# TengdaHan/TemporalAlignNet

Hardware: AMD Instinct MI355X
Metric: video-seq/sec (len=64, E6D6) at 1/2/4/8 MI355X; HTM-Align ROC-AUC parity (higher is better)
Workload: dtype bf16; 1 GPU; E6D6 len=64 bf16 stage-1 (init: multi-positive NCE only) train step (fwd+loss+bwd+AdamW), synthetic HTM-370K-shaped features, N~U[4,16] sentences/video; global_batch=128, per_gpu_batch=128, seq_len=64, parallelism=dp1

## Files before the change

temporalalignnet_amd/csrc/tan_attnblk.hip:

```cpp
#include "tan_panel.h"
#include "tan_attn_img.h"

namespace tal {

typedef float f32x4_t __attribute__((ext_vector_type(4)));

struct AbFwdArgs {
    const bf16_t* xn1; const bf16_t* x_in; const unsigned char* keypad;
    const char* pw_qkv;
    const char* pw_out;
    const float* b_qkv; const float* b_out;
    bf16_t* qkv; bf16_t* attn_o; float* lse;
    bf16_t* x_mid;
    int L, H;
    long long* dbg;
    float* part; long part_plane;
};

constexpr int AB_D = 4;
struct AbWFrags { bf16x8 f[3]; };

__device__ __forceinline__ void ab_load_wa(AbWFrags& W, const char* pw, int hp, int ks, int wave, int lane) {
    const char* p = pw + ((long)((hp * 16 + ks) * PN_WAVES + wave) * 3) * 1024 + lane * 16;
#pragma unroll
    for (int i = 0; i < 3; ++i) W.f[i] = *reinterpret_cast<const bf16x8*>(p + i * 1024);
}
__device__ __forceinline__ void ab_load_wb(AbWFrags& W, const char* pw, int kt, int wave, int lane) {
    const char* p = pw + (long)kt * 16384 + wave * 2048 + lane * 16;
#pragma unroll
    for (int i = 0; i < 2; ++i) W.f[i] = *reinterpret_cast<const bf16x8*>(p + i * 1024);
}

template <int NKB>
__device__ __forceinline__ float ab_attn_unit(char* Qi, const char* Ki, const char* Vi, const float* bias, int q0, int lane) {
    const int c = lane & 31, hh = lane >> 5;
    bf16x8 qf[4];
#pragma unroll
    for (int ks = 0; ks < 4; ++ks) qf[ks] = img_frag_kc(Qi, q0 + c, 2 * ks + hh);
    f32x16 s[NKB];
    float m = -INFINITY;
#pragma unroll
    for (int kb = 0; kb < NKB; ++kb) {
        acc_zero(s[kb]);
#pragma unroll
        for (int ks = 0; ks < 4; ++ks)
            s[kb] = __builtin_amdgcn_mfma_f32_32x32x16_bf16(img_frag_kc(Ki, 32 * kb + c, 2 * ks + hh), qf[ks], s[kb], 0, 0, 0);
#pragma unroll
        for (int g4 = 0; g4 < 4; ++g4) {
            const float4 bv = *reinterpret_cast<const float4*>(bias + 32 * kb + 8 * g4 + 4 * hh);
            const float bb[4] = {bv.x, bv.y, bv.z, bv.w};
#pragma unroll
            for (int e = 0; e < 4; ++e) {
                const float v = s[kb][4 * g4 + e] * 0.125f + bb[e];
                s[kb][4 * g4 + e] = v;
                m = fmaxf(m, v);
            }
        }
    }
    m = fmaxf(m, __shfl_xor(m, 32, 64));
    const bool dead = (m == -INFINITY);
    float sum = 0.f;
#pragma unroll
    for (int kb = 0; kb < NKB; ++kb)
#pragma unroll
        for (int r = 0; r < 16; ++r) {
            const float e = dead ? 0.f : __expf(s[kb][r] - m);
            s[kb][r] = e;
            sum += e;
        }
    sum += __shfl_xor(sum, 32, 64);
    const float inv = dead ? 0.f : 1.0f / sum;
    f32x16 o[2];
    acc_zero(o[0]); acc_zero(o[1]);
#pragma unroll
    for (int kb = 0; kb < NKB; ++kb) {
#pragma unroll
        for (int r = 0; r < 16; ++r) s[kb][r] *= inv;
#pragma unroll
        for (int j = 0; j < 2; ++j) {
            const bf16x8 pf = acc_frag(s[kb], j);
#pragma unroll
            for (int db = 0; db < 2; ++db)
                o[db] = __builtin_amdgcn_mfma_f32_32x32x16_bf16(img_frag_tr(Vi, 32 * kb + 16 * j, 32 * db, lane), pf, o[db], 0, 0, 0);
        }
    }
#pragma unroll
    for (int db = 0; db < 2; ++db)
#pragma unroll
        for (int g4 = 0; g4 < 4; ++g4) {
            const int row = q0 + c, chunk = 4 * db + g4;
            st4((bf16_t*)(Qi + row * 128 + ((chunk ^ img_swz(row)) << 4) + hh * 8),
                make_float4(o[db][4 * g4], o[db][4 * g4 + 1], o[db][4 * g4 + 2], o[db][4 * g4 + 3]));
        }
    return dead ? -INFINITY : m + logf(sum);
}

__device__ __forceinline__ void ab_rows_out(const char* img, int r0, int lane, bf16_t* out, long ld, int L) {
#pragma unroll
    for (int it = 0; it < 4; ++it) {
        const int row = r0 + it * 8 + (lane >> 3), chunk = lane & 7;
        const uint4 v = *reinterpret_cast<const uint4*>(img + row * 128 + ((chunk ^ img_swz(row)) << 4));
        if (row < L) *reinterpret_cast<uint4*>(out + (long)row * ld + chunk * 8) = v;
    }
}

template <int NRB16, bool SPLIT = false>
__global__ __launch_bounds__(64 * PN_WAVES, PN_WAVES / 4) void attnblk_fwd_kernel(AbFwdArgs a) {
    static_assert(PN_WAVES == 8, "eight waves");
    constexpr int NKB = (NRB16 + 1) / 2, LP = 32 * NKB, XROWS = 16 * NRB16, D = AB_D;
    constexpr int XP_OFF = 0, IMG_OFF = XROWS * 1024, IMG_B = LP * 128, BIAS_OFF = IMG_OFF + 6 * IMG_B, BQ_OFF = BIAS_OFF + LP * 4, LDS_B = BQ_OFF + 1536 * 4;
    static_assert(LDS_B <= 163840, "LDS budget");
    __shared__ __attribute__((aligned(1024))) char lds[LDS_B];

    const int tid = threadIdx.x, lane = tid & 63, hi = lane >> 5;
    const int wave = __builtin_amdgcn_readfirstlane(tid >> 6);
    const int L = a.L, C = 512;
    const long row0 = (long)blockIdx.x * L;
    const char* const pwa = a.pw_qkv;
    const char* const pwb = a.pw_out;
    const int hp0 = SPLIT ? (int)blockIdx.y : 0, hp1 = SPLIT ? hp0 + 1 : 4;

    AbWFrags WQ[D];
    pn_static_for<0, D>([&](auto jc) {
        constexpr int J = decltype(jc)::value;
        ab_load_wa(WQ[J], pwa, hp0, J, wave, lane);
    });

    {
        constexpr int RPW = XROWS / PN_WAVES;
        uint4 v[RPW];
#pragma unroll
        for (int r = 0; r < RPW; ++r) {
            const int m = wave * RPW + r;
            v[r] = *reinterpret_cast<const uint4*>(a.xn1 + (row0 + min(m, L - 1)) * C + lane * 8);
        }
#pragma unroll
        for (int r = 0; r < RPW; ++r) *reinterpret_cast<uint4*>(pn_panel_slot<1024>(lds + XP_OFF, wave * RPW + r, lane)) = v[r];
        float* bias = reinterpret_cast<float*>(lds + BIAS_OFF);
        const unsigned char* kp = a.keypad ? a.keypad + (long)blockIdx.x * L : nullptr;
        for (int j = tid; j < LP; j += 64 * PN_WAVES) bias[j] = (j >= L || (kp && kp[j])) ? -INFINITY : 0.f;
        for (int j = tid; j < 1536 / 4; j += 64 * PN_WAVES)
            reinterpret_cast<float4*>(lds + BQ_OFF)[j] = reinterpret_cast<const float4*>(a.b_qkv)[j];
        if constexpr (LP > XROWS) {
            constexpr int PER = (LP - XROWS) * 8;
            for (int i = tid; i < 6 * PER; i += 64 * PN_WAVES)
                *reinterpret_cast<uint4*>(lds + IMG_OFF + (i / PER) * IMG_B + XROWS * 128 + (i % PER) * 16) = make_uint4(0, 0, 0, 0);
        }
    }
    __syncthreads();

    f32x16 acc_o[2][NKB];
#pragma unroll
    for (int i = 0; i < 2; ++i)
#pragma unroll
        for (int j = 0; j < NKB; ++j) acc_zero(acc_o[i][j]);

    typedef __attribute__((address_space(3))) const bf16x8* lds_frag_t;
    const float* bias = reinterpret_cast<const float*>(lds + BIAS_OFF);
    const bool saving = a.qkv != nullptr;

    constexpr int PPI = LP / 8, NPW = 2 * PPI / PN_WAVES;
    constexpr int NIDLE = PN_WAVES - 2 * NKB, NKV = 4 * PPI / NIDLE;
    static_assert(2 * PPI % PN_WAVES == 0 && 4 * PPI % NIDLE == 0, "piece split");
    uint4 cpv;
    auto copy_read = [&](int i, int ln) __attribute__((always_inline)) {
        const int g = wave + PN_WAVES * i, j = g / PPI, row = (g % PPI) * 8 + (ln >> 3), chunk = ln & 7;
        cpv = *reinterpret_cast<const uint4*>(lds + IMG_OFF + (j * 3) * IMG_B + row * 128 + ((chunk ^ img_swz(row)) << 4));
    };
    auto copy_store = [&](int i, int ln, int hp_prev) __attribute__((always_inline)) {
        const int g = wave + PN_WAVES * i, j = g / PPI, row = (g % PPI) * 8 + (ln >> 3), chunk = ln & 7;
        if (row < L) *reinterpret_cast<uint4*>(a.attn_o + (row0 + row) * C + (2 * hp_prev + j) * 64 + chunk * 8) = cpv;
    };

    f32x4_t acc_a[3][NRB16];
    auto gemm_a = [&](int hp, auto copy_flag) __attribute__((always_inline)) {
        constexpr bool COPY = decltype(copy_flag)::value;
        int ln = lane;
        asm volatile("" : "+v"(ln));
        const int xrow = ln & 15, xq = ln >> 4;
        const unsigned xbase = (unsigned)(uintptr_t)(lds + XP_OFF + xrow * 1024);
#pragma unroll
        for (int fb = 0; fb < 3; ++fb) {
            const int p = 3 * wave + fb, which = (p >> 2) % 3, j = p / 12, fblk = p & 3;
            const float4 bv = *reinterpret_cast<const float4*>(lds + BQ_OFF + (which * C + (2 * hp + j) * 64 + fblk * 16 + 4 * xq) * 4);
#pragma unroll
            for (int rb = 0; rb < NRB16; ++rb) { acc_a[fb][rb][0] = bv.x; acc_a[fb][rb][1] = bv.y; acc_a[fb][rb][2] = bv.z; acc_a[fb][rb][3] = bv.w; }
        }
        bf16x8 X[NRB16];
#pragma unroll
        for (int rb = 0; rb < NRB16; ++rb) X[rb] = *(lds_frag_t)(uintptr_t)(xbase + rb * 16384 + ((xq ^ xrow) << 4));
        __builtin_amdgcn_sched_barrier(0);
        pn_static_for<0, 16>([&](auto jc) {
            constexpr int KS = decltype(jc)::value;
            AbWFrags& W = WQ[KS % D];
            if constexpr (COPY) {
                if (saving) {
                    if constexpr (KS >= 1 && KS <= NPW) copy_store(KS - 1, ln, hp - 1);
                    if constexpr (KS < NPW) copy_read(KS, ln);
                }
            }
#pragma unroll
            for (int rb = 0; rb < NRB16; ++rb) {
#pragma unroll
                for (int fb = 0; fb < 3; ++fb)
                    acc_a[fb][rb] = __builtin_amdgcn_mfma_f32_16x16x32_bf16(W.f[fb], X[rb], acc_a[fb][rb], 0, 0, 0);
                if constexpr (KS < 15) X[rb] = *(lds_frag_t)(uintptr_t)(xbase + rb * 16384 + ((((KS + 1) * 4 + xq) ^ xrow) << 4));
            }
            if constexpr (KS + D < 16) ab_load_wa(W, pwa, hp, KS + D, wave, ln);
            else ab_load_wb(W, pwb, hp * 8 + (KS + D - 16), wave, ln);
            __builtin_amdgcn_sched_barrier(0);
        });
    };

    gemm_a(hp0, std::false_type{});
#pragma unroll 1
    for (int hp = hp0; hp < hp1; ++hp) {
        __syncthreads();
        {
            int ln = lane;
            asm volatile("" : "+v"(ln));
            const int erow = ln & 15, eq = ln >> 4;
#pragma unroll
            for (int fb = 0; fb < 3; ++fb) {
                const int p = 3 * wave + fb, which = (p >> 2) % 3, j = p / 12, fblk = p & 3;
                char* img = lds + IMG_OFF + (j * 3 + which) * IMG_B;
#pragma unroll
                for (int rb = 0; rb < NRB16; ++rb) {
                    const int row = rb * 16 + erow, chunk = fblk * 2 + (eq >> 1);
                    uint2 u;
                    u.x = f2bf2(acc_a[fb][rb][0], acc_a[fb][rb][1]);
                    u.y = f2bf2(acc_a[fb][rb][2], acc_a[fb][rb][3]);
                    *reinterpret_cast<uint2*>(img + row * 128 + ((chunk ^ img_swz(row)) << 4) + (eq & 1) * 8) = u;
                }
            }
        }
        __syncthreads();

        if (wave >= 2 * NKB) {
            if (saving) {
                int ln = lane;
                asm volatile("" : "+v"(ln));
#pragma unroll 4
                for (int i = 0; i < NKV; ++i) {
                    const int g = (wave - 2 * NKB) + NIDLE * i, im = g / PPI, j = im >> 1, which = 1 + (im & 1);
                    const int row = (g % PPI) * 8 + (ln >> 3), chunk = ln & 7;
                    const uint4 v = *reinterpret_cast<const uint4*>(lds + IMG_OFF + (j * 3 + which) * IMG_B + row * 128 + ((chunk ^ img_swz(row)) << 4));
                    if (row < L) *reinterpret_cast<uint4*>(a.qkv + (row0 + row) * (3 * C) + which * C + (2 * hp + j) * 64 + chunk * 8) = v;
                }
            }
        } else {
            int ln = lane;
            asm volatile("" : "+v"(ln));
            const int j = wave / NKB, q0 = (wave % NKB) * 32, h = 2 * hp + j;
            char* Qi = lds + IMG_OFF + (j * 3) * IMG_B;
            if (saving) ab_rows_out(Qi, q0, ln, a.qkv + row0 * (3 * C) + h * 64, 3 * C, L);
            const float l = ab_attn_unit<NKB>(Qi, Qi + IMG_B, Qi + 2 * IMG_B, bias, q0, ln);
            if (saving && ln < 32 && q0 + ln < L) a.lse[((long)blockIdx.x * a.H + h) * L + q0 + ln] = l;
        }
        __syncthreads();

        {
            int ln = lane;
            asm volatile("" : "+v"(ln));
            pn_static_for<0, 8>([&](auto jc) {
                constexpr int KB = decltype(jc)::value;
                const char* Oi = lds + IMG_OFF + ((KB >> 2) * 3) * IMG_B;
                AbWFrags& W = WQ[KB % D];
                bf16x8 of[NKB];
#pragma unroll
                for (int rb = 0; rb < NKB; ++rb) of[rb] = img_frag_kc(Oi, rb * 32 + (ln & 31), 2 * (KB & 3) + (ln >> 5));
#pragma unroll
                for (int nb = 0; nb < 2; ++nb)
#pragma unroll
                    for (int rb = 0; rb < NKB; ++rb)
                        acc_o[nb][rb] = __builtin_amdgcn_mfma_f32_32x32x16_bf16(W.f[nb], of[rb], acc_o[nb][rb], 0, 0, 0);
                if constexpr (KB + D < 8) ab_load_wb(W, pwb, hp * 8 + KB + D, wave, ln);
                else if (hp + 1 < hp1) ab_load_wa(W, pwa, hp + 1, KB + D - 8, wave, ln);
                __builtin_amdgcn_sched_barrier(0);
            });
        }
        if (hp + 1 < hp1) gemm_a(hp + 1, std::true_type{});
    }
    if constexpr (SPLIT) {
        if (saving) {
#pragma unroll 1
            for (int i = 0; i < NPW; ++i) { copy_read(i, lane); copy_store(i, lane, hp0); }
        }
#pragma unroll
        for (int nb = 0; nb < 2; ++nb)
#pragma unroll
            for (int mb = 0; mb < NKB; ++mb) {
                const int m = mb * 32 + (lane & 31);
                if (m < L) {
                    float* dst = a.part + hp0 * a.part_plane + (row0 + m) * C + wave * 64 + nb * 32 + 16 * hi;
#pragma unroll
                    for (int q = 0; q < 4; ++q)
                        *reinterpret_cast<float4*>(dst + 4 * q) = make_float4(acc_o[nb][mb][4 * q], acc_o[nb][mb][4 * q + 1], acc_o[nb][mb][4 * q + 2],
                                                                              acc_o[nb][mb][4 * q + 3]);
                }
            }
        return;
    }
    uint4 resq[2][NKB][2];
#pragma unroll
    for (int nb = 0; nb < 2; ++nb)
#pragma unroll
        for (int mb = 0; mb < NKB; ++mb)
#pragma unroll
            for (int p = 0; p < 2; ++p)
                resq[nb][mb][p] = *reinterpret_cast<const uint4*>(a.x_in + (row0 + min(mb * 32 + (lane & 31), L - 1)) * C + wave * 64 + nb * 32 + (2 * hi + p) * 8);
    if (saving) {
#pragma unroll 1
        for (int i = 0; i < NPW; ++i) { copy_read(i, lane); copy_store(i, lane, 3); }
    }

    __syncthreads();
    char* xo_panel = lds + XP_OFF;
#pragma unroll
    for (int nb = 0; nb < 2; ++nb) {
        const int nbase = wave * 64 + nb * 32;
        pn_cfptr_t bp = (pn_cfptr_t)(uintptr_t)(a.b_out) + nbase;
#pragma unroll
        for (int mb = 0; mb < NKB; ++mb) {
            const int m = mb * 32 + (lane & 31);
#pragma unroll
            for (int p = 0; p < 2; ++p) {
                float bias8[8], res[8], v[8];
                pn_uniform8(bp + 8 * p, bp + 16 + 8 * p, hi, bias8);
                pn_unpack8(resq[nb][mb][p], res);
#pragma unroll
                for (int e = 0; e < 8; ++e) v[e] = acc_o[nb][mb][8 * p + e] + bias8[e] + res[e];
                if (m < XROWS) *reinterpret_cast<uint4*>(pn_panel_slot<1024>(xo_panel, m, (nbase >> 3) + 2 * hi + p)) = pn_pack8(v);
            }
        }
    }
    __syncthreads();
    for (int m = wave; m < L; m += PN_WAVES)
        *reinterpret_cast<uint4*>(a.x_mid + (row0 + m) * C + lane * 8) = *reinterpret_cast<const uint4*>(pn_panel_slot<1024>(xo_panel, m, lane));
}

__global__ __launch_bounds__(256) void attnblk_split_finish_kernel(const float* __restrict__ part, long plane, const bf16_t* __restrict__ x_in,
                                                                   const float* __restrict__ b_out, bf16_t* __restrict__ x_mid, long rows) {
    const int lane = threadIdx.x & 63, wave = threadIdx.x >> 6;
    const long row = (long)blockIdx.x * 4 + wave;
    if (row >= rows) return;
    f8 acc = ld8f(part + row * 512 + lane * 8);
#pragma unroll
    for (int c = 1; c < 4; ++c) {
        const f8 t = ld8f(part + c * plane + row * 512 + lane * 8);
#pragma unroll
        for (int j = 0; j < 8; ++j) acc.v[j] += t.v[j];
    }
    const f8 res = ld8(x_in + row * 512 + lane * 8), bias = ld8f(b_out + lane * 8);
    f8 v;
#pragma unroll
    for (int j = 0; j < 8; ++j) v.v[j] = acc.v[j] + bias.v[j] + res.v[j];
    st8(x_mid + row * 512 + lane * 8, v);
}

}

using namespace tal;

static long long* g_ab_dbg = nullptr;
extern "C" int tan_attnblk_lab_set_dbg(void* p) { g_ab_dbg = (long long*)p; return 0; }

extern "C" int tan_attnblk_supported(int L, int C, int H, int dtype) {
    return dtype == TAN_BF16 && C == 512 && H == 8 && L > 48 && L <= 80;
}

extern "C" int tan_attnblk_fwd(const tan_attnblk_desc* d, void* stream) {
    TAN_REQUIRE(d && d->xn1 && d->x_in && d->pw_qkv && d->pw_out && d->b_qkv && d->b_out && d->x_mid && d->B > 0);
    TAN_REQUIRE(tan_attnblk_supported(d->L, d->C, d->H, TAN_BF16));
    TAN_REQUIRE((d->qkv != nullptr) == (d->attn_o != nullptr) && (d->qkv != nullptr) == (d->lse != nullptr));
    AbFwdArgs a;
    a.xn1 = (const bf16_t*)d->xn1; a.x_in = (const bf16_t*)d->x_in; a.keypad = d->key_padding_mask;
    a.pw_qkv = (const char*)d->pw_qkv; a.pw_out = (const char*)d->pw_out; a.b_qkv = d->b_qkv; a.b_out = d->b_out;
    a.qkv = (bf16_t*)d->qkv; a.attn_o = (bf16_t*)d->attn_o; a.lse = d->lse; a.x_mid = (bf16_t*)d->x_mid;
    a.L = d->L; a.H = d->H; a.dbg = g_ab_dbg;
    a.part = nullptr; a.part_plane = 0;
    const dim3 grid((unsigned)d->B);
    const double rows = (double)d->B * d->L;
    const int rec = prof_begin((hipStream_t)stream, TAN_PROF_ATTNBLK, 2.0 * rows * 512.0 * 2048.0 + 4.0 * rows * d->L * 512.0);
    if (d->L <= 64) hipLaunchKernelGGL((attnblk_fwd_kernel<4>), grid, dim3(64 * PN_WAVES), 0, (hipStream_t)stream, a);
    else hipLaunchKernelGGL((attnblk_fwd_kernel<5>), grid, dim3(64 * PN_WAVES), 0, (hipStream_t)stream, a);
    prof_end((hipStream_t)stream, rec);
    TAN_LAUNCH_CHECK();
    return 0;
}

extern "C" int tan_attnblk_fwd_split(const tan_attnblk_desc* d, float* part, void* stream) {
    TAN_REQUIRE(d && part && d->xn1 && d->x_in && d->pw_qkv && d->pw_out && d->b_qkv && d->b_out && d->x_mid && d->B > 0);
    TAN_REQUIRE(tan_attnblk_supported(d->L, d->C, d->H, TAN_BF16));
    TAN_REQUIRE((d->qkv != nullptr) == (d->attn_o != nullptr) && (d->qkv != nullptr) == (d->lse != nullptr));
    AbFwdArgs a;
    a.xn1 = (const bf16_t*)d->xn1; a.x_in = (const bf16_t*)d->x_in; a.keypad = d->key_padding_mask;
    a.pw_qkv = (const char*)d->pw_qkv; a.pw_out = (const char*)d->pw_out; a.b_qkv = d->b_qkv; a.b_out = d->b_out;
    a.qkv = (bf16_t*)d->qkv; a.attn_o = (bf16_t*)d->attn_o; a.lse = d->lse; a.x_mid = (bf16_t*)d->x_mid;
    a.L = d->L; a.H = d->H; a.dbg = nullptr;
    const long rows = (long)d->B * d->L;
    a.part = part; a.part_plane = rows * 512;
    const hipStream_t st = (hipStream_t)stream;
    const dim3 grid((unsigned)d->B, 4);
    const int rec = prof_begin(st, TAN_PROF_ATTNBLK, 2.0 * rows * 512.0 * 2048.0 + 4.0 * rows * d->L * 512.0);
    if (d->L <= 64) hipLaunchKernelGGL((attnblk_fwd_kernel<4, true>), grid, dim3(64 * PN_WAVES), 0, st, a);
    else hipLaunchKernelGGL((attnblk_fwd_kernel<5, true>), grid, dim3(64 * PN_WAVES), 0, st, a);
    prof_end(st, rec);
    TAN_LAUNCH_CHECK();
    hipLaunchKernelGGL(attnblk_split_finish_kernel, dim3(cdiv(rows, 4)), dim3(256), 0, st, part, rows * 512, (const bf16_t*)d->x_in, d->b_out,
                       (bf16_t*)d->x_mid, rows);
    TAN_LAUNCH_CHECK();
    return 0;
}
```

Measured before the change: 31550 video-seq/s.

## Add warp-specialized pipelined attention block kernel overlapping QKV GEMM with attention

Adds a new fused attention-block forward kernel that splits the eight waves into producer and consumer groups. Four waves compute the next head's QKV projection into double-buffered LDS images while the other four run attention for the current head, then all waves accumulate the output projection. Weight fragments for the next stage are prefetched inside the MFMA loops. The new kernel is enabled by default through an environment flag, and it adds LDS pressure and per-head barriers.

```diff
diff --git a/temporalalignnet_amd/csrc/tan_attnblk.hip b/temporalalignnet_amd/csrc/tan_attnblk.hip
--- a/temporalalignnet_amd/csrc/tan_attnblk.hip
+++ b/temporalalignnet_amd/csrc/tan_attnblk.hip
@@ -339,6 +339,226 @@
         *reinterpret_cast<uint4*>(a.x_mid + (row0 + m) * C + lane * 8) = *reinterpret_cast<const uint4*>(pn_panel_slot<1024>(xo_panel, m, lane));
 }
 
+template <int NRB16, bool CLK = false>
+__global__ __launch_bounds__(64 * PN_WAVES, PN_WAVES / 4) void attnblk_fwd_pipe_kernel(AbFwdArgs a) {
+    static_assert(PN_WAVES == 8, "eight waves");
+    constexpr int NKB = (NRB16 + 1) / 2, LP = 32 * NKB, XROWS = 16 * NRB16, D = AB_D, NH = 8;
+    constexpr int XP_OFF = 0, IMG_OFF = XROWS * 1024, IMG_B = LP * 128, BIAS_OFF = IMG_OFF + 6 * IMG_B, BQ_OFF = BIAS_OFF + LP * 4, LDS_B = BQ_OFF + 1536 * 4;
+    static_assert(LDS_B <= 163840, "LDS budget");
+    __shared__ __attribute__((aligned(1024))) char lds[LDS_B];
+
+    const int tid = threadIdx.x, lane = tid & 63, hi = lane >> 5;
+    const int wave = __builtin_amdgcn_readfirstlane(tid >> 6);
+    const bool gw = wave < 4;
+    const int rw = wave & 3;
+    const int L = a.L, C = 512;
+    const long row0 = (long)blockIdx.x * L;
+    const char* const pwa = a.pw_qkv;
+    const char* const pwb = a.pw_out;
+    auto clk = [&](int i) __attribute__((always_inline)) {
+        if constexpr (CLK) {
+            if (blockIdx.x == 0 && lane == 0) a.dbg[wave * 32 + i] = (long long)__builtin_amdgcn_s_memtime();
+        }
+    };
+    clk(0);
+    auto load_wa = [&](AbWFrags& W, int h, int ks, int ln) __attribute__((always_inline)) { ab_load_wa(W, pwa, h >> 1, ks, 4 * (h & 1) + rw, ln); };
+
+    auto load_sel = [&](AbWFrags& W, bool in, int h, int ks, int kt, int ln) __attribute__((always_inline)) {
+        const char* p = in ? pwa + ((long)(((h >> 1) * 16 + ks) * PN_WAVES + 4 * (h & 1) + rw) * 3) * 1024 : pwb + (long)kt * 16384 + wave * 2048;
+        p += ln * 16;
+        const int o2 = in ? 2048 : 1024;
+        W.f[0] = *reinterpret_cast<const bf16x8*>(p);
+        W.f[1] = *reinterpret_cast<const bf16x8*>(p + 1024);
+        W.f[2] = *reinterpret_cast<const bf16x8*>(p + o2);
+    };
+
+    AbWFrags WQ[D];
+    pn_static_for<0, D>([&](auto jc) { load_sel(WQ[decltype(jc)::value], gw, 0, decltype(jc)::value, decltype(jc)::value, lane); });
+
+    {
+        constexpr int RPW = XROWS / PN_WAVES;
+        uint4 v[RPW];
+#pragma unroll
+        for (int r = 0; r < RPW; ++r) {
+            const int m = wave * RPW + r;
+            v[r] = *reinterpret_cast<const uint4*>(a.xn1 + (row0 + min(m, L - 1)) * C + lane * 8);
+        }
+#pragma unroll
+        for (int r = 0; r < RPW; ++r) *reinterpret_cast<uint4*>(pn_panel_slot<1024>(lds + XP_OFF, wave * RPW + r, lane)) = v[r];
+        float* bias = reinterpret_cast<float*>(lds + BIAS_OFF);
+        const unsigned char* kp = a.keypad ? a.keypad + (long)blockIdx.x * L : nullptr;
+        for (int j = tid; j < LP; j += 64 * PN_WAVES) bias[j] = (j >= L || (kp && kp[j])) ? -INFINITY : 0.f;
+        for (int j = tid; j < 1536 / 4; j += 64 * PN_WAVES)
+            reinterpret_cast<float4*>(lds + BQ_OFF)[j] = reinterpret_cast<const float4*>(a.b_qkv)[j];
+        if constexpr (LP > XROWS) {
+            constexpr int PER = (LP - XROWS) * 8;
+            for (int i = tid; i < 6 * PER; i += 64 * PN_WAVES)
+                *reinterpret_cast<uint4*>(lds + IMG_OFF + (i / PER) * IMG_B + XROWS * 128 + (i % PER) * 16) = make_uint4(0, 0, 0, 0);
+        }
+    }
+    __syncthreads();
+    clk(1);
+
+    f32x16 acc_o[2][NKB];
+#pragma unroll
+    for (int i = 0; i < 2; ++i)
+#pragma unroll
+        for (int j = 0; j < NKB; ++j) acc_zero(acc_o[i][j]);
+
+    typedef __attribute__((address_space(3))) const bf16x8* lds_frag_t;
+    const float* bias = reinterpret_cast<const float*>(lds + BIAS_OFF);
+    const bool saving = a.qkv != nullptr;
+
+    f32x4_t acc_a[3][NRB16];
+    auto gemm_a = [&](int h, auto first_flag) __attribute__((always_inline)) {
+        constexpr bool FIRST = decltype(first_flag)::value;
+        int ln = lane;
+        asm volatile("" : "+v"(ln));
+        const int xrow = ln & 15, xq = ln >> 4;
+        const unsigned xbase = (unsigned)(uintptr_t)(lds + XP_OFF + xrow * 1024);
+#pragma unroll
+        for (int fb = 0; fb < 3; ++fb) {
+            const int p = 3 * rw + fb, which = p >> 2, fblk = p & 3;
+            const float4 bv = *reinterpret_cast<const float4*>(lds + BQ_OFF + (which * C + h * 64 + fblk * 16 + 4 * xq) * 4);
+#pragma unroll
+            for (int rb = 0; rb < NRB16; ++rb) { acc_a[fb][rb][0] = bv.x; acc_a[fb][rb][1] = bv.y; acc_a[fb][rb][2] = bv.z; acc_a[fb][rb][3] = bv.w; }
+        }
+        bf16x8 X[NRB16];
+#pragma unroll
+        for (int rb = 0; rb < NRB16; ++rb) X[rb] = *(lds_frag_t)(uintptr_t)(xbase + rb * 16384 + ((xq ^ xrow) << 4));
+        __builtin_amdgcn_sched_barrier(0);
+        pn_static_for<0, 16>([&](auto jc) {
+            constexpr int KS = decltype(jc)::value;
+            AbWFrags& W = WQ[KS % D];
+#pragma unroll
+            for (int rb = 0; rb < NRB16; ++rb) {
+#pragma unroll
+                for (int fb = 0; fb < 3; ++fb)
+                    acc_a[fb][rb] = __builtin_amdgcn_mfma_f32_16x16x32_bf16(W.f[fb], X[rb], acc_a[fb][rb], 0, 0, 0);
+                if constexpr (KS < 15) X[rb] = *(lds_frag_t)(uintptr_t)(xbase + rb * 16384 + ((((KS + 1) * 4 + xq) ^ xrow) << 4));
+            }
+            if constexpr (KS + D < 16) load_wa(W, h, KS + D, ln);
+            else if constexpr (FIRST) load_wa(W, h + 1, KS + D - 16, ln);
+            else ab_load_wb(W, pwb, (h - 1) * 4 + (KS + D - 16), wave, ln);
+            __builtin_amdgcn_sched_barrier(0);
+        });
+    };
+    auto epi_a = [&](int h) __attribute__((always_inline)) {
+        int ln = lane;
+        asm volatile("" : "+v"(ln));
+        const int erow = ln & 15, eq = ln >> 4;
+#pragma unroll
+        for (int fb = 0; fb < 3; ++fb) {
+            const int p = 3 * rw + fb, which = p >> 2, fblk = p & 3;
+            char* img = lds + IMG_OFF + ((h & 1) * 3 + which) * IMG_B;
+#pragma unroll
+            for (int rb = 0; rb < NRB16; ++rb) {
+                const int row = rb * 16 + erow, chunk = fblk * 2 + (eq >> 1);
+                uint2 u;
+                u.x = f2bf2(acc_a[fb][rb][0], acc_a[fb][rb][1]);
+                u.y = f2bf2(acc_a[fb][rb][2], acc_a[fb][rb][3]);
+                *reinterpret_cast<uint2*>(img + row * 128 + ((chunk ^ img_swz(row)) << 4) + (eq & 1) * 8) = u;
+            }
+        }
+    };
+
+    if (gw) {
+        gemm_a(0, std::true_type{});
+        epi_a(0);
+    }
+    __syncthreads();
+    clk(2);
+
+    constexpr int PPI = LP / 8, NIA = 4 - NKB, NKV = 2 * PPI / NIA;
+    static_assert(NIA >= 1 && 2 * PPI % NIA == 0, "piece split");
+#pragma unroll 1
+    for (int h = 0; h < NH; ++h) {
+        char* const Qi = lds + IMG_OFF + ((h & 1) * 3) * IMG_B;
+        if (gw) {
+            if (h + 1 < NH) {
+                gemm_a(h + 1, std::false_type{});
+                epi_a(h + 1);
+            }
+        } else {
+            int ln = lane;
+            asm volatile("" : "+v"(ln));
+            if (rw < NKB) {
+                const int q0 = rw * 32;
+                if (saving) ab_rows_out(Qi, q0, ln, a.qkv + row0 * (3 * C) + h * 64, 3 * C, L);
+                const float l = ab_attn_unit<NKB>(Qi, Qi + IMG_B, Qi + 2 * IMG_B, bias, q0, ln);
+                if (saving) {
+                    if (ln < 32 && q0 + ln < L) a.lse[((long)blockIdx.x * a.H + h) * L + q0 + ln] = l;
+                    rows_to_global(Qi, q0, ln, a.attn_o + row0 * C + h * 64, C, 0, L);
+                }
+            } else if (saving) {
+#pragma unroll 4
+                for (int i = 0; i < NKV; ++i) {
+                    const int g = (rw - NKB) + NIA * i, which = 1 + g / PPI;
+                    const int row = (g % PPI) * 8 + (ln >> 3), chunk = ln & 7;
+                    const uint4 v = *reinterpret_cast<const uint4*>(Qi + which * IMG_B + row * 128 + ((chunk ^ img_swz(row)) << 4));
+                    if (row < L) *reinterpret_cast<uint4*>(a.qkv + (row0 + row) * (3 * C) + which * C + h * 64 + chunk * 8) = v;
+                }
+            }
+        }
+        clk(3 + 3 * h);
+        __syncthreads();
+        clk(4 + 3 * h);
+
+        {
+            int ln = lane;
+            asm volatile("" : "+v"(ln));
+            pn_static_for<0, 4>([&](auto jc) {
+                constexpr int KB = decltype(jc)::value;
+                AbWFrags& W = WQ[KB];
+                bf16x8 of[NKB];
+#pragma unroll
+                for (int rb = 0; rb < NKB; ++rb) of[rb] = img_frag_kc(Qi, rb * 32 + (ln & 31), 2 * KB + (ln >> 5));
+#pragma unroll
+                for (int nb = 0; nb < 2; ++nb)
+#pragma unroll
+                    for (int rb = 0; rb < NKB; ++rb)
+                        acc_o[nb][rb] = __builtin_amdgcn_mfma_f32_32x32x16_bf16(W.f[nb], of[rb], acc_o[nb][rb], 0, 0, 0);
+                load_sel(W, gw && h + 2 < NH, h + 2, KB, min(h + 1, NH - 1) * 4 + KB, ln);
+                __builtin_amdgcn_sched_barrier(0);
+            });
+        }
+        clk(5 + 3 * h);
+        __syncthreads();
+    }
+
+    uint4 resq[2][NKB][2];
+#pragma unroll
+    for (int nb = 0; nb < 2; ++nb)
+#pragma unroll
+        for (int mb = 0; mb < NKB; ++mb)
+#pragma unroll
+            for (int p = 0; p < 2; ++p)
+                resq[nb][mb][p] = *reinterpret_cast<const uint4*>(a.x_in + (row0 + min(mb * 32 + (lane & 31), L - 1)) * C + wave * 64 + nb * 32 + (2 * hi + p) * 8);
+    char* xo_panel = lds + XP_OFF;
+#pragma unroll
+    for (int nb = 0; nb < 2; ++nb) {
+        const int nbase = wave * 64 + nb * 32;
+        pn_cfptr_t bp = (pn_cfptr_t)(uintptr_t)(a.b_out) + nbase;
+#pragma unroll
+        for (int mb = 0; mb < NKB; ++mb) {
+            const int m = mb * 32 + (lane & 31);
+#pragma unroll
+            for (int p = 0; p < 2; ++p) {
+                float bias8[8], res[8], v[8];
+                pn_uniform8(bp + 8 * p, bp + 16 + 8 * p, hi, bias8);
+                pn_unpack8(resq[nb][mb][p], res);
+#pragma unroll
+                for (int e = 0; e < 8; ++e) v[e] = acc_o[nb][mb][8 * p + e] + bias8[e] + res[e];
+                if (m < XROWS) *reinterpret_cast<uint4*>(pn_panel_slot<1024>(xo_panel, m, (nbase >> 3) + 2 * hi + p)) = pn_pack8(v);
+            }
+        }
+    }
+    __syncthreads();
+    for (int m = wave; m < L; m += PN_WAVES)
+        *reinterpret_cast<uint4*>(a.x_mid + (row0 + m) * C + lane * 8) = *reinterpret_cast<const uint4*>(pn_panel_slot<1024>(xo_panel, m, lane));
+    clk(30);
+}
+
 __global__ __launch_bounds__(256) void attnblk_split_finish_kernel(const float* __restrict__ part, long plane, const bf16_t* __restrict__ x_in,
                                                                    const float* __restrict__ b_out, bf16_t* __restrict__ x_mid, long rows) {
     const int lane = threadIdx.x & 63, wave = threadIdx.x >> 6;
@@ -364,6 +584,11 @@
 
 static long long* g_ab_dbg = nullptr;
 extern "C" int tan_attnblk_lab_set_dbg(void* p) { g_ab_dbg = (long long*)p; return 0; }
+
+static bool attnblk_pipe() {
+    static const int on = [] { const char* e = getenv("TAN_ATTNBLK_PIPE"); return e ? atoi(e) : 1; }();
+    return on != 0;
+}
 
 extern "C" int tan_attnblk_supported(int L, int C, int H, int dtype) {
     return dtype == TAN_BF16 && C == 512 && H == 8 && L > 48 && L <= 80;
@@ -382,8 +607,18 @@
     const dim3 grid((unsigned)d->B);
     const double rows = (double)d->B * d->L;
     const int rec = prof_begin((hipStream_t)stream, TAN_PROF_ATTNBLK, 2.0 * rows * 512.0 * 2048.0 + 4.0 * rows * d->L * 512.0);
-    if (d->L <= 64) hipLaunchKernelGGL((attnblk_fwd_kernel<4>), grid, dim3(64 * PN_WAVES), 0, (hipStream_t)stream, a);
-    else hipLaunchKernelGGL((attnblk_fwd_kernel<5>), grid, dim3(64 * PN_WAVES), 0, (hipStream_t)stream, a);
+    const hipStream_t st = (hipStream_t)stream;
+    const dim3 block(64 * PN_WAVES);
+    if (!attnblk_pipe()) {
+        if (d->L <= 64) hipLaunchKernelGGL((attnblk_fwd_kernel<4>), grid, block, 0, st, a);
+        else hipLaunchKernelGGL((attnblk_fwd_kernel<5>), grid, block, 0, st, a);
+    } else if (a.dbg) {
+        if (d->L <= 64) hipLaunchKernelGGL((attnblk_fwd_pipe_kernel<4, true>), grid, block, 0, st, a);
+        else hipLaunchKernelGGL((attnblk_fwd_pipe_kernel<5, true>), grid, block, 0, st, a);
+    } else {
+        if (d->L <= 64) hipLaunchKernelGGL((attnblk_fwd_pipe_kernel<4>), grid, block, 0, st, a);
+        else hipLaunchKernelGGL((attnblk_fwd_pipe_kernel<5>), grid, block, 0, st, a);
+    }
     prof_end((hipStream_t)stream, rec);
     TAN_LAUNCH_CHECK();
     return 0;
```

Result: faster. 32010 video-seq/s, median of 6 (+1.5%).
